# cage-challenge/cage-challenge-4

Hardware: AMD Instinct MI355X
Metric: agent-env steps/sec (5 blue agents x N envs) (higher is better)
Workload: dtype int32

## Files before the change

cage_challenge_4_amd/csrc/cc4_engine.h:

```cpp
#pragma once
#include "cc4_state.h"
#include "cc4_tables.h"

namespace cc4 {

struct Ctx { EnvState* s; EnvCold* c; Rng* r; HostDyn* hd; StepWork* w; unsigned long long* prof = nullptr;
             unsigned long long* aprof = nullptr; EvLog* lg = nullptr; const uint64_t* gpre = nullptr;
             const ExtAct* ext = nullptr; };

#if defined(__HIP_DEVICE_COMPILE__)
#define CC4_TICK(x, i) do { if ((x).prof) { unsigned long long _t = clock64(); (x).prof[(i)] += _t - (x).prof[15]; (x).prof[15] = _t; } } while (0)
#define CC4_TICK0(x) do { if ((x).prof) (x).prof[15] = clock64(); } while (0)
#define CC4_AT0(x) unsigned long long _at = (x).aprof ? clock64() : 0
#define CC4_AT(x, k) do { if ((x).aprof) { unsigned long long _n = clock64(); (x).aprof[(k)] += _n - _at; _at = _n; } } while (0)
#if defined(CC4_FINE)
#define CC4_FT0(x, r) unsigned long long _ft = ((x).aprof && (r) == 0) ? clock64() : 0
#define CC4_FT(x, r, k) do { if ((x).aprof && (r) == 0) { unsigned long long _n = clock64(); (x).aprof[88 + (k)] += _n - _ft; _ft = _n; } } while (0)
#else
#define CC4_FT0(x, r) do { } while (0)
#define CC4_FT(x, r, k) do { } while (0)
#endif
#else
#define CC4_FT0(x, r) do { } while (0)
#define CC4_FT(x, r, k) do { } while (0)
// ... 246 lines not shown
}
CC4_HD void step_red_merge(Ctx x) {
  EnvState* s = x.s;
  uint32_t pr[NRED];
  CC4_UNROLL for (int r = 0; r < NRED; ++r) pr[r] = x.w->pend_r[r];
  CC4_UNROLL for (int r = 0; r < NRED; ++r) {
    if (!pr[r]) continue;
    if (s->npend >= MAX_PEND) set_err(x, E_PEND_OVERFLOW); else s->pend[s->npend++] = pr[r];
    x.w->pend_r[r] = 0;
  }
}
CC4_HD void pend_drop_host(Ctx x, int h) {
  EnvState* s = x.s;
  int n = 0;
  for (int i = 0; i < s->npend; ++i) if ((int)(s->pend[i] >> 16) != h) s->pend[n++] = s->pend[i];
  s->npend = (uint8_t)n;
}
CC4_HD bool subnet_blocked(Ctx x, int src_sub, int other_sub) { return (x.s->blocks[other_sub] >> src_sub) & 1u; }

struct S8 { uint64_t v[8]; uint64_t slots; };
CC4_HD uint64_t rs_word(const EnvState* s, int slot) { uint64_t v; __builtin_memcpy(&v, &s->spool[slot], 8); return v; }
CC4_HD void rs_word_put(EnvState* s, int slot, uint64_t v) { __builtin_memcpy(&s->spool[slot], &v, 8); }
CC4_HD S8 rs_load8(const EnvState* s, const RedAgent& a, int i0) {
  S8 q;
  __builtin_memcpy(&q.slots, &a.sord[i0], 8);
  CC4_UNROLL for (int k = 0; k < 8; ++k) q.v[k] = rs_word(s, (int)((q.slots >> (8 * k)) & 0xFF));
  return q;
}
CC4_HD int s8_slot(const S8& q, int k) { return (int)((q.slots >> (8 * k)) & 0xFF); }
CC4_HD int rsw_id(uint64_t v) { return (int)(v & 0xFFFF); }
CC4_HD int rsw_pid(uint64_t v) { return (int)((v >> 16) & 0xFFFF); }
CC4_HD int rsw_host(uint64_t v) { return (int)((v >> 32) & 0xFF); }
CC4_HD int rsw_flags(uint64_t v) { return (int)((v >> 40) & 0xFF); }
CC4_HD uint64_t rsw_make(int id, int pid, int host, int flags) {
  return (uint64_t)(id & 0xFFFF) | ((uint64_t)(pid & 0xFFFF) << 16) | ((uint64_t)(host & 0xFF) << 32) | ((uint64_t)(flags & 0xFF) << 40);
}
CC4_HD uint64_t rs_at(const EnvState* s, const RedAgent& a, int i) { return rs_word(s, a.sord[i]); }
CC4_HD int rs_find_id(const EnvState* s, const RedAgent& a, int id, int n) {
  for (int i0 = 0; i0 < n; i0 += 8) {
    const S8 q = rs_load8(s, a, i0);
    int hit = -1;
    CC4_UNROLL for (int k = 7; k >= 0; --k) if (i0 + k < n && rsw_id(q.v[k]) == id) hit = i0 + k;
    if (hit >= 0) return hit;
  }
  return -1;
}
CC4_HD int rs_find_id(const EnvState* s, const RedAgent& a, int id) { return rs_find_id(s, a, id, a.h.nsess); }
struct HostSess { int n, first, first_root; };
CC4_HD HostSess rs_on_host(const EnvState* s, const RedAgent& a, int h) {
  HostSess r; r.n = 0; r.first = -1; r.first_root = -1;
  const int n = a.h.nsess;
  for (int i0 = 0; i0 < n; i0 += 8) {
    const S8 q = rs_load8(s, a, i0);
    CC4_UNROLL for (int k = 0; k < 8; ++k)
      if (i0 + k < n && rsw_host(q.v[k]) == h) {
        r.n++;
        if (r.first < 0) r.first = i0 + k;
        if (r.first_root < 0 && (rsw_flags(q.v[k]) & RS_ROOT)) r.first_root = i0 + k;
      }
  }
  return r;
}
CC4_HD int rs_kth_on_host(const EnvState* s, const RedAgent& a, int h, int kth) {
  const int n = a.h.nsess;
  for (int i0 = 0; i0 < n; i0 += 8) {
    const S8 q = rs_load8(s, a, i0);
    int hit = -1;
    CC4_UNROLL for (int k = 0; k < 8; ++k)
      if (hit < 0 && i0 + k < n && rsw_host(q.v[k]) == h) { if (kth == 0) hit = i0 + k; kth--; }
    if (hit >= 0) return hit;
  }
  return -1;
}
CC4_HD int rs_find_host_pid(const EnvState* s, const RedAgent& a, int h, int pid) {
  const int n = a.h.nsess;
  for (int i0 = 0; i0 < n; i0 += 8) {
    const S8 q = rs_load8(s, a, i0);
    int hit = -1;
    CC4_UNROLL for (int k = 7; k >= 0; --k) if (i0 + k < n && rsw_host(q.v[k]) == h && rsw_pid(q.v[k]) == pid) hit = i0 + k;
    if (hit >= 0) return hit;
  }
  return -1;
}
CC4_HD void rs_list_remove(RedAgent& a, int idx) {
  uint64_t w[MAX_RS / 8];
  __builtin_memcpy(w, a.sord, MAX_RS);
  const int wi = idx >> 3, sh = 8 * (idx & 7);
  CC4_UNROLL for (int k = 0; k < MAX_RS / 8; ++k) {
    if (k < wi) continue;
    const uint64_t nxt = k + 1 < MAX_RS / 8 ? w[k + 1] : 0ull;
    uint64_t v = (w[k] >> 8) | (nxt << 56);
    if (k == wi && sh) v = (w[k] & ((1ull << sh) - 1ull)) | (v & ~((1ull << sh) - 1ull));
    w[k] = v;
  }
  __builtin_memcpy(a.sord, w, MAX_RS);
}
CC4_HD int rs_alloc_lowest(Ctx x) {
  for (int w = 0; w < RS_POOL / 32; ++w) {
    const uint32_t fr = ~x.s->spool_used[w];
    if (fr) return w * 32 + ctz32(fr);
  }
  return -1;
}
CC4_HD void rs_reserve(Ctx x) {
  uint32_t used[RS_POOL / 32];
  CC4_UNROLL for (int w = 0; w < RS_POOL / 32; ++w) used[w] = x.s->spool_used[w];
  int ty[NRED];
  CC4_UNROLL for (int r = 0; r < NRED; ++r) ty[r] = x.s->rexec[r].type;
  CC4_UNROLL for (int r = 0; r < NRED; ++r) {
    int slot = 0xFF;
    if (ty[r] == RA_EXPLOIT) {
      CC4_UNROLL for (int w = 0; w < RS_POOL / 32; ++w) {
        const uint32_t fr = ~used[w];
        if (slot == 0xFF && fr) { slot = w * 32 + ctz32(fr); used[w] |= 1u << (slot & 31); }
      }
    }
    x.w->rs_slot[r] = (uint8_t)slot;
  }
}
CC4_HD int rs_add(Ctx x, int r, int host, int pid, int flags, int slot = -1) {
  EnvState* s = x.s;
  RedAgent& a = s->red[r];
  if (slot < 0) slot = rs_alloc_lowest(x);
  if (a.h.nsess >= MAX_RS || slot < 0 || slot >= RS_POOL) { set_err(x, E_RSESS_OVERFLOW); return -1; }
  int id = 0;
  for (int i0 = 0; i0 < a.h.nsess; i0 += 8) {
    const S8 q = rs_load8(s, a, i0);
    CC4_UNROLL for (int k = 0; k < 8; ++k) if (i0 + k < a.h.nsess && rsw_id(q.v[k]) + 1 > id) id = rsw_id(q.v[k]) + 1;
  }
  (void)or_shared(&s->spool_used[slot >> 5], 1u << (slot & 31));
  rs_word_put(s, slot, rsw_make(id, pid, host, flags));
  if (flags & RS_ABSTRACT) {
    uint64_t* row = reinterpret_cast<uint64_t*>(x.c->kports[slot]);
    for (int k = 0; k < (MAXH + 7) / 8; ++k) row[k] = 0;
  }
  a.sord[a.h.nsess++] = (uint8_t)slot;
  a.h.rsc_dirty = 1; a.h.fsm_dirty = 1;
  if (!bit_get(a.live_hosts, host)) { bit_set(a.live_hosts, host); a.h.nlive++; }
  bit_set_shared(s->red_hosts, host);
  return a.h.nsess - 1;
}
CC4_HD void rs_host_left(Ctx x, int r, int gone) {
  RedAgent& a = x.s->red[r];
  bit_clr(a.live_hosts, gone); a.h.nlive--;
  uint32_t lw[NRED];
  CC4_UNROLL for (int q = 0; q < NRED; ++q) lw[q] = x.s->red[q].live_hosts[gone >> 5];
  uint32_t any_other = 0;
  CC4_UNROLL for (int q = 0; q < NRED; ++q) any_other |= lw[q];
  if (!((any_other >> (gone & 31)) & 1u)) bit_clr_shared(x.s->red_hosts, gone);
}
CC4_HD void rs_remove_at(Ctx x, int r, int idx, bool keep_record = false) {
  EnvState* s = x.s;
  RedAgent& a = s->red[r];
  const int slot = a.sord[idx];
  const int gone = rsw_host(rs_word(s, slot));
  if (!keep_record) bit_clr_shared(s->spool_used, slot);
  rs_list_remove(a, idx);
  a.h.nsess--;
  a.h.rsc_dirty = 1; a.h.fsm_dirty = 1;
  if (rs_on_host(s, a, gone).n == 0) rs_host_left(x, r, gone);
}
CC4_HD void rs_remove_on_host(Ctx x, int r, int h) {
  EnvState* s = x.s;
  RedAgent& a = s->red[r];
  const int n = a.h.nsess;
  int out = 0, removed = 0;
// ... 751 lines not shown
    CC4_UNROLL for (int r = 0; r < NRED; ++r) nc += nl[r];
    if (nc == 0) return;
    int c = (int)rng_below(x.r, (uint32_t)nc);
    CC4_UNROLL for (int w = 0; w < 5; ++w) {
      uint32_t m = rh[w];
      if (src >= 0 || !m) continue;
      int inw = 0;
      CC4_UNROLL for (int r = 0; r < NRED; ++r) inw += popc32(lh[r][w]);
      if (c >= inw) { c -= inw; continue; }
      while (m && src < 0) {
        int b = ctz32(m); m &= m - 1;
        CC4_UNROLL for (int r = 0; r < NRED; ++r)
          if (src < 0 && ((lh[r][w] >> b) & 1u)) { if (c-- == 0) src = r; }
      }
    }
  }
  const P8N hd0 = proc_head(x, gh);
  int pid = create_pid(x, gh, hd0);
  if (!add_proc_n(x, gh, hd0.n, pid, K_SESS_RED, 0)) return;
  rs_add(x, src, gh, pid, RS_ABSTRACT);
}
CC4_HD uint64_t green_prepare(Ctx x, int g, int act) {
  EnvState* s = x.s;
  const int gh = s->green_host[g];
  uint64_t w = 0;
  if (act == 1) {
    const HostDyn& d = x.hd[gh];
    uint32_t sv[MAXSV];
    __builtin_memcpy(sv, d.svcs, sizeof(sv));
    const int nsvc = hd_nsvc(d);
    CC4_UNROLL for (int i = 0; i < MAXSV; ++i) if (i < nsvc) w |= (uint64_t)(sv[i] >> 24) << (8 * i);
  } else if (act == 0) {
    uint32_t allowed = green_allowed_mask(s->phase, h_subnet(gh));
    if (x.ext && x.ext[NRED + g].type == XG_ACCESS && x.ext[NRED + g].sid) {
      allowed = (uint32_t)x.ext[NRED + g].sid;
      if (!((allowed >> h_subnet(gh)) & 1u)) allowed = 1u << h_subnet(gh);
    }
    uint64_t ns;
    __builtin_memcpy(&ns, s->n_servers, 8);
    int n = 0;
    CC4_UNROLL for (int sn = 0; sn < NSUB - 1; ++sn) { if ((allowed >> sn) & 1u) n += (int)((ns >> (8 * sn)) & 0xFF); w |= (uint64_t)n << (8 * sn); }
  }
  return w;
}
CC4_HD int green_as_dest(uint64_t pre, int c, int* sn_out) {
  int sn = 0, before = 0;
  CC4_UNROLL for (int k = 0; k < NSUB - 2; ++k) { const int tot = (int)((pre >> (8 * k)) & 0xFF); if (tot <= c) { sn = k + 1; before = tot; } }
  *sn_out = sn;
  return h_make(sn, 11 + (c - before));
}
CC4_HD uint32_t green_lw_active(uint64_t pre) {
  uint32_t act = 0;
  CC4_UNROLL for (int i = 0; i < MAXSV; ++i) if ((pre >> (8 * i)) & SV_ACTIVE) act |= 1u << i;
  return act;
}
CC4_HD bool green_local_work(Ctx x, int gh, uint64_t pre, bool* want_phish, double fp_rate = 0.01, double phish_rate = 0.01) {
  const uint32_t act = green_lw_active(pre);
  if (!act) return false;
  const int c = nth_bit(act, (int)rng_below(x.r, (uint32_t)popc32(act)));
  const uint32_t st = (uint32_t)(pre >> (8 * c)) & 0xFF;
  int rel = (int)(st & 0x7F) * 20;
  if ((int)rng_below(x.r, 100) >= rel) return false;
  if (rng_random_lt(x.r, fp_rate)) { int port = eph_port(x, gh); ev_proc(x, gh, 0); ev_log(x, gh, gh, 1, gh, port, 0xFF, 0, 0); }
  if (rng_random_lt(x.r, phish_rate)) *want_phish = true;
  return true;
}
CC4_HD bool green_access_service(Ctx x, int gh, uint64_t pre, double fp_rate = 0.01) {
  int own = h_subnet(gh);
  const int n = (int)(pre >> 56);
  const int c = (int)rng_below(x.r, (uint32_t)n);
  int sn;
  const int dest = green_as_dest(pre, c, &sn);
  const int dest_port = eph_port(x, dest);
  int ds = sn;
  if (subnet_blocked(x, ds, own) || subnet_blocked(x, own, ds)) { ev_conn(x, dest); ev_log(x, gh, dest, 0, dest, 0, gh, 8800, 0); return false; }
  if (rng_random_lt(x.r, fp_rate)) { ev_conn(x, dest); ev_log(x, gh, dest, 0, gh, 0, dest, dest_port, 0); }
  return true;
}

CC4_HD void red_result(Ctx x, int r, const Act& a, int success) {
  int arg = a.type == RA_DRS ? a.arg : 0;
  obs_first(x, r, success, a.type, a.host, arg);
}
CC4_HD void red_drs(Ctx x, int r, const Act& a) {
  EnvState* s = x.s;
  int sn = a.arg; bool any = false;
  if (rs_find_id(s, s->red[r], a.sid) < 0) { red_result(x, r, a, T_FALSE); return; }
  bool allowed = (red_allowed_mask(r) >> sn) & 1u;
  RedAgent& A = s->red[r];
  const int lo = sn * SLOTS + 1, w0 = lo >> 5, off = lo & 31, w1 = (w0 + 1 < 5) ? w0 + 1 : w0;
  const uint32_t e0 = s->exists[w0], e1 = s->exists[w1], h0 = A.obs_has[1][w0], h1 = A.obs_has[1][w1];
  auto field = [&](uint32_t a0, uint32_t a1) { uint32_t v = a0 >> off; if (off > 16 && w1 != w0) v |= a1 << (32 - off); return v & 0xFFFFu; };
  const uint32_t ex = field(e0, e1);
  any = ex != 0;
  if (allowed && ex) {
    const uint32_t had = field(h0, h1) & ex;
    uint32_t fresh = ex & ~had;
    const uint32_t m0 = ex << off, m1 = (off > 16 && w1 != w0) ? ex >> (32 - off) : 0u;
    A.as_ip[w0] |= m0; A.obs_has[1][w0] = h0 | m0;
    if (m1) { A.as_ip[w1] |= m1; A.obs_has[1][w1] = h1 | m1; }
    A.h.as_subnet |= (uint16_t)(1u << sn);
    int n = A.h.nobs;
    while (fresh) {
      const int b = ctz32(fresh); fresh &= fresh - 1;
      if (n >= MAX_OBS) { set_err(x, E_OBS_OVERFLOW); break; }
      A.obs[n].host = (uint8_t)(lo + b); A.obs[n].flags = (uint8_t)(OE_IFACE | OE_KEY_IP);
      n++;
    }
    A.h.nobs = (uint8_t)n;
    uint32_t again = had;
    while (again) { const int b = ctz32(again); again &= again - 1; obs_put(x, r, true, lo + b, OE_IFACE, true); }
  }
  red_result(x, r, a, any ? T_TRUE : T_UNKNOWN);
}
CC4_HD int port_of_bit(int pb) { return pb == PB_22 ? 22 : (pb == PB_80 ? 80 : (pb == PB_3390 ? 3390 : (pb == PB_25 ? 25 : (pb == PB_1 ? 1 : 443)))); }
CC4_HD void red_scan(Ctx x, int r, const Act& a, double rate) {
  EnvState* s = x.s;
  RedAgent& A = s->red[r];
  int si = rs_find_id(s, A, a.sid);
  if (si < 0) { red_result(x, r, a, T_FALSE); return; }
  const int slot = A.sord[si];
  const uint64_t sw = rs_word(s, slot);
  if (!(rsw_flags(sw) & RS_ABSTRACT)) { red_result(x, r, a, T_FALSE); return; }
  int src = rsw_host(sw), tgt = a.host;
  if (subnet_blocked(x, h_subnet(src), h_subnet(tgt))) { red_result(x, r, a, T_FALSE); return; }
  const bool fixed_le_rate = rng_random_le(x.r, rate);
  int ports = 0;
  const P8N hd0 = proc_head(x, tgt);
  const int np = hd0.n;
  for (int i0 = 0; i0 < np; i0 += 8) {
    P8 q = p8_of(hd0);
    if (i0) q = proc_load8(x, tgt, i0);
    CC4_UNROLL for (int k8 = 0; k8 < 8; ++k8) {
      if (i0 + k8 >= np) continue;
      int k = pw_kind(q.v[k8]);
      int pb = kind_port(k);
      if (!pb) continue;
      ports |= pb;
      if (fixed_le_rate || kind_is_decoy(k)) { ev_conn(x, tgt); int ep = eph_port(x, tgt, (i0 + k8) & 63); ev_log(x, 200 + r, tgt, 0, tgt, port_of_bit(pb), src, ep, 0); }
    }
  }
  if (ports) {
    obs_put(x, r, true, tgt, OE_IFACE, false);
    x.c->kports[slot][tgt] = (uint8_t)(PB_HAS | ports);
  }
  red_result(x, r, a, T_TRUE);
}
CC4_HD int exploit_new_session(Ctx x, int r, int parent_sid, int tgt, const P8N& hd0) {
  (void)parent_sid;
  int pid = create_pid(x, tgt, hd0);
  if (!add_proc_n(x, tgt, hd0.n, pid, K_SHELL, 0)) return -1;
  x.hd[tgt].nsf = (uint8_t)((hd0.nsf & 0x0F) | ((((hd0.nsf >> 4) | HF_CMD) & ~HF_ESC_LAST) << 4));
  return rs_add(x, r, tgt, pid, RS_CHILD, x.w->rs_slot[r]);
}
CC4_HD void red_exploit(Ctx x, int r, const Act& a) {
  EnvState* s = x.s;
  RedAgent& A = s->red[r];
  int si = rs_find_id(s, A, a.sid);
  if (si < 0) { red_result(x, r, a, T_FALSE); return; }
  const int slot = A.sord[si];
  const uint64_t sw = rs_word(s, slot);
  if (!(rsw_flags(sw) & RS_ABSTRACT)) { red_result(x, r, a, T_FALSE); return; }
  int src = rsw_host(sw), tgt = a.host;
  const P8N thd0 = proc_head(x, tgt);
  int known = x.c->kports[slot][tgt];
  if (!(known & PB_HAS)) { red_result(x, r, a, T_FALSE); return; }
  if (subnet_blocked(x, h_subnet(src), h_subnet(tgt))) { red_result(x, r, a, T_FALSE); return; }
  enum { X_HTTPRFI = 0, X_HTTPSRFI = 1, X_SSH = 2, X_SQLI = 3, X_HARAKA = 4 };
  uint32_t opts = 0;
  if (known & PB_80) opts |= 1u << X_HTTPRFI;
  if (known & PB_443) opts |= 1u << X_HTTPSRFI;
  if (known & PB_22) opts |= 1u << X_SSH;
  if ((known & PB_3390) && (known & (PB_80 | PB_443))) opts |= 1u << X_SQLI;
  if (known & PB_25) opts |= 1u << X_HARAKA;
  if (opts == 0) { red_result(x, r, a, T_FALSE); return; }
  int sel = ctz32(opts);
  if (popc32(opts) > 1) {
    int top = (opts >> X_HARAKA) & 1u ? X_HARAKA : ((opts >> X_SQLI) & 1u ? X_SQLI : ((opts >> X_HTTPSRFI) & 1u ? X_HTTPSRFI : X_HTTPRFI));
    opts &= ~(1u << top);
    sel = nth_bit(opts, (int)rng_below(x.r, (uint32_t)popc32(opts)));
    (void)rng_random(x.r);
  }
  const int tnp = thd0.n;
  if (sel == X_SSH) {
    uint8_t* work = reinterpret_cast<uint8_t*>(x.w->scratch + 6 * r);
    int nh = route(src, tgt, work);
    for (int i = 0; i < nh; ++i) if (!rng_random_le(x.r, 0.050000000000000044)) { ev_conn(x, work[12 + i]); ev_log(x, 200 + r, work[12 + i], 0, tgt, 0, src, 22, 0); }
    int vp = -1;
    for (int i0 = 0; i0 < tnp && vp < 0; i0 += 8) {
      P8 q = p8_of(thd0);
      if (i0) q = proc_load8(x, tgt, i0);
      CC4_UNROLL for (int k = 7; k >= 0; --k) if (i0 + k < tnp && pw_kind(q.v[k]) == K_SSHD) vp = i0 + k;
    }
    if (vp < 0) { red_result(x, r, a, T_FALSE); return; }
    obs_put(x, r, true, tgt, OE_IFACE, false);
    const int bf_port = eph_port(x, tgt);
    ev_conn(x, tgt);
    ev_log(x, 200 + r, tgt, 0, tgt, 22, src, bf_port, 0, 10);
    int ni = exploit_new_session(x, r, a.sid, tgt, thd0);
    if (ni < 0) { red_result(x, r, a, T_FALSE); return; }
    const uint64_t nw = rs_at(s, A, ni);
    ev_proc_red(x, r, tgt, rsw_pid(nw));
    ev_log(x, 200 + r, tgt, 1, 0xFF, 0, 0xFF, 0, rsw_pid(nw));
    obs_put(x, r, true, tgt, OE_SESS | OE_IFACE | OE_SYSHN, false);
    obs_put(x, r, true, src, OE_IFACE, false);
    A.h.new_sess_host = (uint8_t)tgt; A.h.new_sess_id = (uint16_t)rsw_id(nw);
    red_result(x, r, a, T_TRUE);
    return;
  }
  int vp = -1, vk = 0;
  {
    const uint32_t want = sel == X_HTTPRFI ? ((1u << K_APACHE) | (1u << K_DEC_APACHE) | (1u << K_DEC_VSFTPD))
                        : sel == X_HTTPSRFI ? (1u << K_DEC_TOMCAT)
                        : sel == X_SQLI ? (1u << K_MYSQL)
                        : ((1u << K_SMTP) | (1u << K_DEC_HARAKA));
    for (int i0 = 0; i0 < tnp && vp < 0; i0 += 8) {
      P8 q = p8_of(thd0);
      if (i0) q = proc_load8(x, tgt, i0);
      CC4_UNROLL for (int k = 7; k >= 0; --k) if (i0 + k < tnp && ((want >> pw_kind(q.v[k])) & 1u)) { vp = i0 + k; vk = pw_kind(q.v[k]); }
    }
  }
  if (vp < 0) { red_result(x, r, a, T_FALSE); return; }
  bool decoy = kind_is_decoy(vk);
  const int xport = sel == X_HTTPRFI ? 80 : (sel == X_HTTPSRFI ? 443 : (sel == X_SQLI ? 3390 : 25));
  if (decoy) { ev_conn(x, tgt); int ep = eph_port(x, tgt, 1); ev_log(x, 200 + r, tgt, 0, tgt, xport, src, ep, 0); }
  obs_put(x, r, true, tgt, OE_IFACE, false);
  bool works = (sel == X_SQLI) || decoy;
  if (!works) { red_result(x, r, a, T_FALSE); return; }
  if (rng_random_le(x.r, 0.0)) { red_result(x, r, a, T_FALSE); return; }
  const int lport = eph_port(x, tgt, 2);
  if (decoy) { ev_conn(x, tgt); int ep = eph_port(x, tgt, 3); ev_log(x, 200 + r, tgt, 0, tgt, lport, src, ep, 0); red_result(x, r, a, T_FALSE); return; }
  int ni = exploit_new_session(x, r, a.sid, tgt, thd0);
  if (ni < 0) { red_result(x, r, a, T_FALSE); return; }
  const uint64_t nw = rs_at(s, A, ni);
  if (!rng_random_le(x.r, 0.050000000000000044)) { ev_proc_red(x, r, tgt, rsw_pid(nw)); ev_log(x, 200 + r, tgt, 1, 0xFF, 0, 0xFF, 0, rsw_pid(nw)); }
  obs_put(x, r, true, tgt, OE_SESS | OE_IFACE | OE_SYSHN, false);
  obs_put(x, r, true, src, OE_IFACE, false);
  A.h.new_sess_host = (uint8_t)tgt; A.h.new_sess_id = (uint16_t)rsw_id(nw);
  red_result(x, r, a, T_TRUE);
}
CC4_HD void red_privesc(Ctx x, int r, const Act& a) {
  EnvState* s = x.s;
  RedAgent& A = s->red[r];
  int h = a.host;
  const HostSess hs = rs_on_host(s, A, h);
  const int n = hs.n;
  int target = hs.first_root;
  if (n == 0) { red_result(x, r, a, T_FALSE); return; }
  if (target < 0) {
    target = rs_kth_on_host(s, A, h, (int)rng_below(x.r, (uint32_t)n));
    { int ss = rs_find_id(s, A, a.sid);
      if (ss < 0 || !(rsw_flags(rs_at(s, A, ss)) & RS_ABSTRACT)) { red_result(x, r, a, T_FALSE); return; } }
    const int tslot = A.sord[target];
    s->spool[tslot].flags |= RS_ROOT;
    hd_touch(x, h);
    hd_set_files(x.hd[h], hd_files(x.hd[h]) | HF_ESC | HF_ESC_LAST);
    int pi = find_proc(x, h, s->spool[tslot].pid);
    if (pi >= 0) proc_put(x, h, pi, proc_get(x, h, pi) | ((uint32_t)PF_ROOT << 24));
  }
  obs_put(x, r, false, h, OE_SESS, false);
  { const uint64_t tw = rs_at(s, A, target); if (rsw_flags(tw) & RS_ABSTRACT) as_know_sid(x, r, rsw_id(tw)); }
  if (rs_find_id(s, A, a.sid) >= 0 && h_slot(h) == 11) {
    uint32_t m = info_links(h_subnet(h));
    for (int sn = 0; sn < NSUB; ++sn) if ((m >> sn) & 1u) obs_put(x, r, false, h_make(sn, 11), OE_IFACE, false);
  }
  red_result(x, r, a, T_TRUE);
}
CC4_HD void red_impact(Ctx x, int r, const Act& a) {
  EnvState* s = x.s;
  RedAgent& A = s->red[r];
  int h = a.host;
  if (rs_on_host(s, A, h).first_root < 0) { red_result(x, r, a, T_FALSE); return; }
  HostDyn& d = x.hd[h];
  const SvTab sv = svc_load(d);
  int si = -1;
  uint32_t sw = 0;
  CC4_UNROLL for (int i = MAXSV - 1; i >= 0; --i) if (i < sv.n && svw_kind(sv.w[i]) == K_OT && (svw_st(sv.w[i]) & SV_ACTIVE)) { si = i; sw = sv.w[i]; }
  if (si < 0) { red_result(x, r, a, T_FALSE); return; }
  if (rs_find_id(s, A, a.sid) < 0) { red_result(x, r, a, T_FALSE); return; }
  hd_touch(x, h);
  d.svcs[si].st = (uint8_t)(svw_st(sw) & ~SV_ACTIVE);
  int pi = find_proc(x, h, (int)(sw & 0xFFFF));
  if (pi >= 0) remove_proc_at(x, h, pi);
  obs_put(x, r, false, h, 0, false);
  red_result(x, r, a, T_TRUE);
}
CC4_HD void red_degrade(Ctx x, int r, const Act& a) {
  EnvState* s = x.s;
  RedAgent& A = s->red[r];
  int h = a.host;
  if (rs_on_host(s, A, h).first_root < 0) { red_result(x, r, a, T_FALSE); return; }
  HostDyn& d = x.hd[h];
  int n = 0;
  hd_touch(x, h);
  const SvTab sv = svc_load(d);
  CC4_UNROLL for (int i = 0; i < MAXSV; ++i) if (i < sv.n && (svw_st(sv.w[i]) & SV_ACTIVE)) {
    n++;
    int rel = svw_st(sv.w[i]) & 0x7F;
    if (rel > 0) rel--;
    d.svcs[i].st = (uint8_t)(SV_ACTIVE | rel);
  }
  if (n == 0) { red_result(x, r, a, T_FALSE); return; }
  obs_put(x, r, false, h, 0, false);
  red_result(x, r, a, T_TRUE);
}
CC4_HD void red_deception(Ctx x, int r, const Act& a) {
  EnvState* s = x.s;
  RedAgent& A = s->red[r];
  if (rs_find_id(s, A, a.sid) < 0) { red_result(x, r, a, T_FALSE); return; }
  int tgt = a.host;
  const double det_rate = (x.ext && (a.busy & AQ_RATE0)) ? x.c->xrate[r][0] : 0.5;
  const double fp_rate = (x.ext && (a.busy & AQ_RATE1)) ? x.c->xrate[r][1] : 0.1;
  const P8N hd0 = proc_head(x, tgt);
  const int np = hd0.n;
  for (int i0 = 0; i0 < np; i0 += 8) {
    P8 q = p8_of(hd0);
    if (i0) q = proc_load8(x, tgt, i0);
    CC4_UNROLL for (int k = 0; k < 8; ++k) {
      if (i0 + k >= np) continue;
      bool decoy = kind_is_decoy(pw_kind(q.v[k]));
      bool rep = false;
      if (rng_random_le(x.r, det_rate) && decoy) rep = true;
      else if (rng_random_le(x.r, fp_rate) && !decoy) rep = true;
      if (rep) obs_put(x, r, false, tgt, OE_IFACE, false);
    }
  }
  red_result(x, r, a, T_TRUE);
}
CC4_HD void red_session_check(Ctx x, int r) {
  EnvState* s = x.s;
  RedAgent& A = s->red[r];
  obs_first(x, r, T_TRUE, RA_NONE, 0, 0);
  if (A.h.nsess == 0) return;
  if (rsw_id(rs_at(s, A, 0)) != 0 && rsw_id(rs_at(s, A, A.h.nsess - 1)) != 0 && rs_find_id(s, A, 0) < 0) {
    int c = (int)rng_below(x.r, (uint32_t)A.h.nsess);
    rs_move_to_end(s, A, c, 0);
    for (int i = 0; i < A.h.nsess; ++i) s->spool[A.sord[i]].flags &= (uint8_t)~RS_CHILD;
  }
  A.h.rsc_listed = 1;
  if (!A.h.rsc_dirty) return;
  const B5 live = b5_load(A.live_hosts);
  { const B5 ip = b5_load(A.as_ip), hn = b5_load(A.as_hn); b5_store(A.as_ip, b5_or(ip, live)); b5_store(A.as_hn, b5_or(hn, live)); }
  {
    uint32_t sub = 0;
    CC4_UNROLL for (int sn = 0; sn < NSUB; ++sn) {
      const int lo = sn * SLOTS, w = lo >> 5, off = lo & 31;
      uint32_t bits = live.w[w] >> off;
      if (off > 32 - SLOTS && w + 1 < 5) bits |= live.w[w + 1] << (32 - off);
      if (bits & ((1u << SLOTS) - 1u)) sub |= 1u << sn;
    }
    A.h.as_subnet |= (uint16_t)sub;
  }
  const int n = A.h.nsess;
  for (int i0 = 0; i0 < n; i0 += 8) {
    const S8 q = rs_load8(s, A, i0);
    uint32_t kw[8];
    CC4_UNROLL for (int k = 0; k < 8; ++k) kw[k] = A.known_bm[(rsw_id(q.v[k]) >> 5) & 7];
    CC4_UNROLL for (int k = 0; k < 8; ++k) {
      if (i0 + k >= n || !(rsw_flags(q.v[k]) & RS_ABSTRACT)) continue;
      const int id = rsw_id(q.v[k]);
      if (id < 256 && ((kw[k] >> (id & 31)) & 1u)) continue;
      as_know_sid(x, r, id);
    }
  }
  A.h.rsc_dirty = 0;
}
CC4_HD void red_withdraw(Ctx x, int r, const Act& a) {
  EnvState* s = x.s;
  RedAgent& A = s->red[r];
  if (rs_find_id(s, A, a.sid) < 0) { red_result(x, r, a, T_FALSE); return; }
  const int h = a.arg;
  uint16_t* ids = reinterpret_cast<uint16_t*>(x.w->scratch + 36);
  int n = 0;
  const int cap = (int)((sizeof(x.w->scratch) - 36 * 4) / 2);
  for (int pass = 0; pass < 2; ++pass)
    for (int i = 0; i < A.h.nsess; ++i) {
      const uint64_t w = rs_at(s, A, i);
      if (rsw_host(w) != h) continue;
      bool child = (rsw_flags(w) & RS_CHILD) != 0;
      if ((pass == 0 && child) || (pass == 1 && !child && rsw_id(w) != 0)) { if (n < cap) ids[n++] = (uint16_t)rsw_id(w); else set_err(x, E_RSESS_OVERFLOW); }
    }
  { int self = rs_find_id(s, A, a.sid); if (rsw_host(rs_at(s, A, self)) == h) { if (n < cap) ids[n++] = (uint16_t)a.sid; else set_err(x, E_RSESS_OVERFLOW); } }
  if (n == 0) { red_result(x, r, a, T_FALSE); return; }
  int ok = T_FALSE;
  for (int k = 0; k < n; ++k) {
    int self = rs_find_id(s, A, a.sid), ti = rs_find_id(s, A, ids[k]);
    if (self < 0 || ti < 0) { ok = T_FALSE; break; }
    int pid = rsw_pid(rs_at(s, A, ti));
    int pi = find_proc(x, h, pid);
    if (pi < 0) { ok = T_FALSE; break; }
    kill_process(x, h, pi, proc_get(x, h, pi));
    ok = T_TRUE;
  }
  red_result(x, r, a, ok);
}
CC4_HD void red_execute(Ctx x, int r, const Act& a) {
  switch (a.type) {
    case RA_DRS: red_drs(x, r, a); break;
    case RA_AGGR: red_scan(x, r, a, (x.ext && (a.busy & AQ_RATE0)) ? x.c->xrate[r][0] : 0.75); break;
    case RA_STEALTH: red_scan(x, r, a, (x.ext && (a.busy & AQ_RATE0)) ? x.c->xrate[r][0] : 0.25); break;
    case RA_DECEPTION: red_deception(x, r, a); break;
    case RA_EXPLOIT: red_exploit(x, r, a); break;
    case RA_PRIVESC: red_privesc(x, r, a); break;
    case RA_IMPACT: red_impact(x, r, a); break;
    case RA_DEGRADE: red_degrade(x, r, a); break;
    case RA_INVALID: obs_first(x, r, T_FALSE, RA_NONE, 0, 0); break;
    case RA_WITHDRAW: red_withdraw(x, r, a); break;
    default: obs_first(x, r, T_UNKNOWN, RA_NONE, 0, 0); break;
  }
}

CC4_HD int fsm_next(int cur, int act, bool success) {
  uint64_t row;
  if (success) switch (cur) {
    case FS_K: row = 0xffffff221ull; break;  case FS_KD: row = 0xffffff331ull; break;
    case FS_S: row = 0xffff42ff3ull; break;  case FS_SD: row = 0xffff53ff3ull; break;
    case FS_U: row = 0x2ff6ffff5ull; break;  case FS_UD: row = 0x3ff7ffff5ull; break;
    case FS_R: row = 0x266fffff7ull; break;  case FS_RD: row = 0x377fffff7ull; break;
    default: row = 0xffffffff8ull; break;
  } else switch (cur) {
    case FS_K: row = 0xffffff000ull; break;  case FS_KD: row = 0xffffff111ull; break;
    case FS_S: row = 0xffff22ff2ull; break;  case FS_SD: row = 0xffff33ff3ull; break;
    case FS_U: row = 0x4ff4ffff4ull; break;  case FS_UD: row = 0x5ff5ffff5ull; break;
    case FS_R: row = 0x666fffff6ull; break;  case FS_RD: row = 0x777fffff7ull; break;
    default: row = 0xffffffff8ull; break;
  }
  int v = (int)((row >> (4 * act)) & 0xF);
  return v == 0xF ? 0xFF : v;
}
CC4_HD int fsm_get(const RedAgent& A, int h) {
  const int v = (A.fsm_st4[h >> 1] >> (4 * (h & 1))) & 0xF;
  return v ? v - 1 : FS_NONE;
}
CC4_HD void fsm_put(RedAgent& A, int h, int st) {
  const int sh = 4 * (h & 1);
  A.fsm_st4[h >> 1] = (uint8_t)((A.fsm_st4[h >> 1] & ~(0xF << sh)) | ((st + 1) << sh));
}
CC4_HD void fsm_set_state(RedAgent& A, int h, int st) {
  if (st >= FS_U && st <= FS_RD) bit_set(A.fsm_ur, h); else bit_clr(A.fsm_ur, h);
  if ((st & 1) || st == FS_F) bit_set(A.fsm_nodrs, h); else bit_clr(A.fsm_nodrs, h);
  fsm_put(A, h, st);
}
CC4_HD void fsm_apply(Ctx x, int r, RedHdr& H, int h, int act, bool success) {
  RedAgent& A = x.s->red[r];
  int cur = fsm_get(A, h);
  if (cur == FS_NONE) return;
  int nx = fsm_next(cur, act, success);
  if (nx == FS_U) nx = ((red_allowed_mask(r) >> h_subnet(h)) & 1u) ? FS_U : FS_F;
  if (nx == 0xFF) nx = cur;
  if (nx != cur) fsm_set_state(A, h, nx);
  if (nx == FS_F && cur != FS_F) {
    int n = 0;
    for (int i = 0; i < H.fsm_n; ++i) if (A.fsm_order[i] != h) A.fsm_order[n++] = A.fsm_order[i];
    H.fsm_n = (uint8_t)n;
  }
}
CC4_HD void fsm_observe(Ctx x, int r, RedHdr& H) {
  RedAgent& A = x.s->red[r];
  CC4_AT0(x);
  if (H.obs_success == T_IN_PROGRESS && H.nobs == 0 && H.rsc_listed && !H.fsm_dirty) return;
  if (H.obs_act_type <= RA_WITHDRAW && H.obs_success != T_IN_PROGRESS && H.obs_success != 0) {
    bool ok = H.obs_success == T_TRUE;
    int t = H.obs_act_type;
    if (t == RA_DRS) {
      const int lo = H.obs_act_arg * SLOTS, hi = lo + SLOTS - 1;
      for (int w = lo >> 5; w <= (hi >> 5) && w < 5; ++w) {
        uint32_t m = A.fsm_known[w];
        if (ok) m &= ~A.fsm_nodrs[w];
        const int l = lo - 32 * w, u = hi - 32 * w;
        if (l > 0) m &= 0xFFFFFFFFu << l;
        if (u < 31) m &= (2u << u) - 1u;
        while (m) { int b = ctz32(m); m &= m - 1; fsm_apply(x, r, H, w * 32 + b, t, ok); }
      }
    } else if (t == RA_PRIVESC || t == RA_IMPACT || t == RA_DEGRADE) {
      int h = H.obs_act_host;
      if (bit_get(A.fsm_known, h) && bit_get(A.fsm_hn, h)) fsm_apply(x, r, H, h, t, ok);
    } else {
      fsm_apply(x, r, H, H.obs_act_host, t, ok);
    }
  }
  CC4_AT(x, 3);
  B5 seen = b5_zero();
  for (int i = 0; i < H.nobs; ++i) {
    int h = A.obs[i].host; int f = A.obs[i].flags;
    if (f & OE_SESS) b5_set(seen, h);
    bool hn = !(f & OE_KEY_IP) || (f & OE_SYSHN);
    bool ip = (f & OE_KEY_IP) || (f & OE_IFACE);
    if (!ip) {
      if (!(bit_get(A.fsm_known, h) && bit_get(A.fsm_hn, h))) { set_err(x, E_UNREACHABLE); }
      continue;
// ... 797 lines not shown
```

cage_challenge_4_amd/csrc/cc4_philox1_body.h:

```cpp
#pragma once
#include "cc4_kernels.h"

#if defined(CC4_EXP_RESET_CALL)
__device__ __attribute__((noinline))
#else
__device__ __forceinline__
#endif
void philox1_autoreset(const StepArgs& a, const int e, const int lane, EnvState* s, HostDyn* const hd, EnvCold* const cold_e, StepWork& work) {
    uint32_t* const ws = a.reset_ws + (size_t)e * RESET_WS_WORDS;
    reset_zero(s, hd, cold_e, lane, WAVE);
    __syncthreads();
    Rng rr; ResetCarry carry; carry.env_key = 0;
    Ctx xm{s, cold_e, &rr, hd, &work};
    if (lane == 0) { rr = s->rng; rr.mode = 1; carry = reset_topology(xm, 0, a.steps, true, a.policy, a.topo, ws, true); }
    __syncthreads();
    Rng rh; rng_fork(&rh, &s->rng, ST_GEN_HOST); rh.mode = 1;
    Ctx xh{s, cold_e, &rh, hd, &work};
    for (int h = lane; h < MAXH; h += WAVE) reset_gen_host(xh, h);
    __syncthreads();
    if (lane == 0) { reset_pid_serial(xm, reset_used_set(s)); reset_agents(xm); }
    __syncthreads();
    reset_used_clear(s, lane, WAVE);
    __syncthreads();
    for (int h = lane; h < MAXH; h += WAVE) reset_host_sessions(xh, h);
// ... 87 lines not shown
      if (is_red) {
        unsigned long long t0 = ap ? clock64() : 0;
        const int dropped = step_red_policy_tick(xr, lane, false, pre_rp);
        if (ap) ap[0] += clock64() - t0;
        if (dropped) atomicSub(&s->n_actions, 1);
      } else if (lane >= 8 && lane < 8 + NBLUE && !(CC4_STOP_ON && a.dbg_stop == 3)) {
        const int b = lane - 8;
        int32_t act = !a.actions ? -1 : a.act_sys ? __hip_atomic_load(a.actions + e * NBLUE + b, __ATOMIC_RELAXED, __HIP_MEMORY_SCOPE_SYSTEM) : a.actions[e * NBLUE + b];
        if (a.rand_out) { act = (int32_t)(((uint64_t)brand * (uint32_t)(b == 4 ? ACT_LONG : ACT_SHORT)) >> 32); a.rand_out[e * NBLUE + b] = act; }
        step_blue_submit(xg, b, act);
        step_tick_blue(xg, b);
        if (!msgs_clean) step_messages(s, a.msgs ? a.msgs + e * NBLUE * MSG_LEN : nullptr, b);
      }
      if (!(CC4_STOP_ON && (a.dbg_stop == 3 || a.dbg_stop == 4))) {
        if (lane < ng) step_green_policy(xg, lane);
        if (lane + WAVE < ng) step_green_policy(xg, lane + WAVE, bank);
      }
      __syncthreads();
      CC4_TICK(x0, 2);
      CC4_STOP(3); CC4_STOP(4); CC4_STOP(5);
      {
        const bool indep = blue_exec_independent(s);
        if (lane == 0) CC4_TICK(x0, 3);
        uint32_t c[4];
        bank_fetch(BK_BEXE, c);
        Ctx xb = xg;
        if (!indep) xb.prof = x0.prof;
        const int rounds = indep ? 1 : 2 * NBLUE;
#pragma nounroll
        for (int i = 0; i < rounds; ++i) {
          int b = lane;
          bool go = lane < NBLUE;
          if (!indep) {
            b = i < NBLUE ? i : i - NBLUE;
            const int ty = s->bexec[b].type;
            go = lane == 0 && ((ty == BA_BLOCK || ty == BA_ALLOW) == (i < NBLUE));
          }
          if (go) {
            rng_set_stream(&rl, ST_BLUE_EXE + (uint32_t)b);
            if (indep) rng_preload(&rl, c);
            blue_execute(xb, b, s->bexec[b]);
          }
        }
        __syncthreads();
        if (lane == 0) CC4_TICK(x0, 5);
      }
      CC4_STOP(6);
      {
        int pen = 0;
        const uint32_t act0 = lane < ng ? work.green_act[lane] : 2u, act1 = lane + WAVE < ng ? work.green_act[lane + WAVE] : 2u;
        const unsigned long long m0 = __ballot(act0 < 2u), m1 = __ballot(act1 < 2u);
        const unsigned long long lt = (1ull << lane) - 1ull;
        const int n0 = __popcll(m0), nact = n0 + __popcll(m1);
        uint8_t* const glist = reinterpret_cast<uint8_t*>(work.scratch);
        static_assert(sizeof(work.scratch) >= MAXG, "the green list fits the scratch words");
        if (act0 < 2u) glist[__popcll(m0 & lt)] = (uint8_t)lane;
        if (act1 < 2u) glist[n0 + __popcll(m1 & lt)] = (uint8_t)(lane + WAVE);
        __syncthreads();
        for (int i = lane; i < nact; i += WAVE) {
          const int g = glist[i];
          uint32_t c[4]; rng_block(&rl, ST_GREEN_EXE + (uint32_t)g, 0, c);
          pen += step_green_exec(xg, g, c);
        }
        if (pen) atomicAdd(&s->brm, pen);
      }
      __syncthreads();
      CC4_TICK(x0, 6);
      CC4_STOP(7);
      if (lane == 0) { step_phishing(x0); CC4_TICK(x0, 1); rs_reserve(x0); conflict_lds = (int)red_conflict_mask(s); if (prof && conflict_lds) prof[4] += 1000000; }
      __syncthreads();
      const uint32_t serial_red = (uint32_t)conflict_lds;
      CC4_STOP(8);
      uint32_t pre_re[4];
      bank_fetch(BK_REXE, pre_re);
      {
        uint32_t todo = serial_red;
        bool side = true;
#pragma nounroll
        for (;;) {
          int r = lane;
          bool go = is_red && !((serial_red >> lane) & 1u);
          Ctx xe = xr;
          if (!side) { r = __ffs((int)todo) - 1; todo &= todo - 1u; go = lane == 0; xe.prof = x0.prof; xe.aprof = nullptr; }
          if (go) {
            unsigned long long t0 = xe.aprof ? clock64() : 0;
            if (s->rexec[r].type != RA_NONE) {
              rng_set_stream(&rl, ST_RED_EXE + (uint32_t)r);
              if (side) rng_preload(&rl, pre_re);
              red_execute(xe, r, s->rexec[r]);
            }
            if (xe.aprof) xe.aprof[1] += clock64() - t0;
          }
          __syncthreads();
          side = false;
          if (!todo) break;
        }
      }
      CC4_STOP(9);
      if (lane == 0) {
        step_red_merge(x0);
        CC4_TICK(x0, 7);
        step_reassign(x0, red_foreign_agents(s));
        CC4_TICK(x0, 8);
      }
      CC4_STOP(10);
      monitor_roll_all(s, lane);
      __syncthreads();
      CC4_TICK(x0, 9);
      CC4_STOP(11);
      if (is_red) { unsigned long long t0 = ap ? clock64() : 0; step_rsc(xr, lane); if (ap) ap[2] += clock64() - t0; }
      if (lane == WAVE - 1) {
        step_monitor_pend(xg);
        step_end(xg, nullptr, false);
        a.reward[e] = s->reward; a.done[e] = s->done;
      }
      CC4_TICK(x0, 10);
    } else if (lane == 0) { a.reward[e] = s->reward; a.done[e] = s->done; }
  }
  __syncthreads();
  CC4_STOP(12);
  unsigned long long t_obs = a.prof ? clock64() : 0;
  {
    int32_t* o = a.obs + (size_t)e * OBS_TOTAL;
    const uint32_t dirty = (do_reset || (a.full_obs && (!PERSIST || item_k == 0))) ? (uint32_t)OD_ALL : (uint32_t)s->obs_dirty;
    encode_obs_fast<WAVE>(s, o, nullptr, false, lane, msgs_clean && !do_reset && dirty != (uint32_t)OD_ALL);
    encode_obs_slow(s, o, dirty, lane);
  }
  __syncthreads();
  CC4_STOP(13);
  if (lane == 0) a.err[e] = s->err;
  unsigned long long t_out = a.prof ? clock64() : 0;
  if (prof && lane == 0) prof[12] += t_out - t_obs;
  if (last) stage_out<HOT_VEC>(reinterpret_cast<uint4*>(a.st + e), lds, lane);
  if (a.obs8) {
    asm volatile("s_waitcnt vmcnt(0)" ::: "memory");
    pack_row_from_obs(a.obs8 + (size_t)e * OBS_PACKED, a.obs + (size_t)e * OBS_TOTAL, lane);
  }
  if (prof && lane == 0) { prof[13] += clock64() - t_out; prof[14] += clock64() - t_begin; }
  if (prof) { __syncthreads(); if (lane < 15) a.prof[PROF_SLOTS * (size_t)e + lane] += prof_lds[lane]; }
}
```

Measured before the change: 1.378 billion.

## Precompute red session lookups cooperatively across the wave before executing red actions

Adds a wave-cooperative query in which groups of 8 lanes scan one red agent's session list in parallel using ballots. From that scan it derives the session index for the action's sid and per-host session counts and first-root positions. The results are passed into each red action handler, replacing that handler's serial per-lane `rs_find_id` and `rs_on_host` scans. This costs an extra wave-wide pass with cross-lane permutes and ballots on the parallel red-execute path, even for agents whose actions never use the lookup.

```diff
diff --git a/cage_challenge_4_amd/csrc/cc4_engine.h b/cage_challenge_4_amd/csrc/cc4_engine.h
--- a/cage_challenge_4_amd/csrc/cc4_engine.h
+++ b/cage_challenge_4_amd/csrc/cc4_engine.h
@@ -352,6 +352,30 @@
   }
   return -1;
 }
+struct RedPre { int si = -1; HostSess hs = {0, -1, -1}; bool ok = false; };
+#if defined(__HIPCC__)
+__device__ __forceinline__ RedPre rs_wave_query(const EnvState* s, int lane, int sid, int host) {
+  const int r = lane >> 3, k = lane & 7, ra = r < NRED ? r : 0;
+  const RedAgent& A = s->red[ra];
+  const int ksid = __builtin_amdgcn_ds_bpermute(ra << 2, sid), khost = __builtin_amdgcn_ds_bpermute(ra << 2, host);
+  const int n = (r < NRED && ksid >= 0) ? (int)A.h.nsess : 0;
+  const int sh = 8 * k;
+  RedPre p; p.ok = true;
+  for (int i0 = 0; __ballot(i0 < n); i0 += 8) {
+    const bool v = i0 + k < n;
+    uint64_t w = 0;
+    if (v) w = rs_word(s, A.sord[i0 + k]);
+    const bool on = v && rsw_host(w) == khost;
+    const uint32_t bid = (uint32_t)(__ballot(v && rsw_id(w) == ksid) >> sh) & 0xFFu;
+    const uint32_t bh = (uint32_t)(__ballot(on) >> sh) & 0xFFu, br = (uint32_t)(__ballot(on && (rsw_flags(w) & RS_ROOT)) >> sh) & 0xFFu;
+    if (p.si < 0 && bid) p.si = i0 + ctz32(bid);
+    p.hs.n += __popc(bh);
+    if (p.hs.first < 0 && bh) p.hs.first = i0 + ctz32(bh);
+    if (p.hs.first_root < 0 && br) p.hs.first_root = i0 + ctz32(br);
+  }
+  return p;
+}
+#endif
 CC4_HD void rs_list_remove(RedAgent& a, int idx) {
   uint64_t w[MAX_RS / 8];
   __builtin_memcpy(w, a.sord, MAX_RS);
@@ -1269,10 +1293,10 @@
   int arg = a.type == RA_DRS ? a.arg : 0;
   obs_first(x, r, success, a.type, a.host, arg);
 }
-CC4_HD void red_drs(Ctx x, int r, const Act& a) {
+CC4_HD void red_drs(Ctx x, int r, const Act& a, RedPre pre = RedPre()) {
   EnvState* s = x.s;
   int sn = a.arg; bool any = false;
-  if (rs_find_id(s, s->red[r], a.sid) < 0) { red_result(x, r, a, T_FALSE); return; }
+  if ((pre.ok ? pre.si : rs_find_id(s, s->red[r], a.sid)) < 0) { red_result(x, r, a, T_FALSE); return; }
   bool allowed = (red_allowed_mask(r) >> sn) & 1u;
   RedAgent& A = s->red[r];
   const int lo = sn * SLOTS + 1, w0 = lo >> 5, off = lo & 31, w1 = (w0 + 1 < 5) ? w0 + 1 : w0;
@@ -1301,10 +1325,10 @@
   red_result(x, r, a, any ? T_TRUE : T_UNKNOWN);
 }
 CC4_HD int port_of_bit(int pb) { return pb == PB_22 ? 22 : (pb == PB_80 ? 80 : (pb == PB_3390 ? 3390 : (pb == PB_25 ? 25 : (pb == PB_1 ? 1 : 443)))); }
-CC4_HD void red_scan(Ctx x, int r, const Act& a, double rate) {
+CC4_HD void red_scan(Ctx x, int r, const Act& a, double rate, RedPre pre = RedPre()) {
   EnvState* s = x.s;
   RedAgent& A = s->red[r];
-  int si = rs_find_id(s, A, a.sid);
+  int si = pre.ok ? pre.si : rs_find_id(s, A, a.sid);
   if (si < 0) { red_result(x, r, a, T_FALSE); return; }
   const int slot = A.sord[si];
   const uint64_t sw = rs_word(s, slot);
@@ -1340,10 +1364,10 @@
   x.hd[tgt].nsf = (uint8_t)((hd0.nsf & 0x0F) | ((((hd0.nsf >> 4) | HF_CMD) & ~HF_ESC_LAST) << 4));
   return rs_add(x, r, tgt, pid, RS_CHILD, x.w->rs_slot[r]);
 }
-CC4_HD void red_exploit(Ctx x, int r, const Act& a) {
+CC4_HD void red_exploit(Ctx x, int r, const Act& a, RedPre pre = RedPre()) {
   EnvState* s = x.s;
   RedAgent& A = s->red[r];
-  int si = rs_find_id(s, A, a.sid);
+  int si = pre.ok ? pre.si : rs_find_id(s, A, a.sid);
   if (si < 0) { red_result(x, r, a, T_FALSE); return; }
   const int slot = A.sord[si];
   const uint64_t sw = rs_word(s, slot);
@@ -1426,17 +1450,17 @@
   A.h.new_sess_host = (uint8_t)tgt; A.h.new_sess_id = (uint16_t)rsw_id(nw);
   red_result(x, r, a, T_TRUE);
 }
-CC4_HD void red_privesc(Ctx x, int r, const Act& a) {
+CC4_HD void red_privesc(Ctx x, int r, const Act& a, RedPre pre = RedPre()) {
   EnvState* s = x.s;
   RedAgent& A = s->red[r];
   int h = a.host;
-  const HostSess hs = rs_on_host(s, A, h);
+  const HostSess hs = pre.ok ? pre.hs : rs_on_host(s, A, h);
   const int n = hs.n;
   int target = hs.first_root;
   if (n == 0) { red_result(x, r, a, T_FALSE); return; }
   if (target < 0) {
     target = rs_kth_on_host(s, A, h, (int)rng_below(x.r, (uint32_t)n));
-    { int ss = rs_find_id(s, A, a.sid);
+    { int ss = pre.ok ? pre.si : rs_find_id(s, A, a.sid);
       if (ss < 0 || !(rsw_flags(rs_at(s, A, ss)) & RS_ABSTRACT)) { red_result(x, r, a, T_FALSE); return; } }
     const int tslot = A.sord[target];
     s->spool[tslot].flags |= RS_ROOT;
@@ -1447,24 +1471,24 @@
   }
   obs_put(x, r, false, h, OE_SESS, false);
   { const uint64_t tw = rs_at(s, A, target); if (rsw_flags(tw) & RS_ABSTRACT) as_know_sid(x, r, rsw_id(tw)); }
-  if (rs_find_id(s, A, a.sid) >= 0 && h_slot(h) == 11) {
+  if ((pre.ok ? pre.si : rs_find_id(s, A, a.sid)) >= 0 && h_slot(h) == 11) {
     uint32_t m = info_links(h_subnet(h));
     for (int sn = 0; sn < NSUB; ++sn) if ((m >> sn) & 1u) obs_put(x, r, false, h_make(sn, 11), OE_IFACE, false);
   }
   red_result(x, r, a, T_TRUE);
 }
-CC4_HD void red_impact(Ctx x, int r, const Act& a) {
+CC4_HD void red_impact(Ctx x, int r, const Act& a, RedPre pre = RedPre()) {
   EnvState* s = x.s;
   RedAgent& A = s->red[r];
   int h = a.host;
-  if (rs_on_host(s, A, h).first_root < 0) { red_result(x, r, a, T_FALSE); return; }
+  if ((pre.ok ? pre.hs : rs_on_host(s, A, h)).first_root < 0) { red_result(x, r, a, T_FALSE); return; }
   HostDyn& d = x.hd[h];
   const SvTab sv = svc_load(d);
   int si = -1;
   uint32_t sw = 0;
   CC4_UNROLL for (int i = MAXSV - 1; i >= 0; --i) if (i < sv.n && svw_kind(sv.w[i]) == K_OT && (svw_st(sv.w[i]) & SV_ACTIVE)) { si = i; sw = sv.w[i]; }
   if (si < 0) { red_result(x, r, a, T_FALSE); return; }
-  if (rs_find_id(s, A, a.sid) < 0) { red_result(x, r, a, T_FALSE); return; }
+  if ((pre.ok ? pre.si : rs_find_id(s, A, a.sid)) < 0) { red_result(x, r, a, T_FALSE); return; }
   hd_touch(x, h);
   d.svcs[si].st = (uint8_t)(svw_st(sw) & ~SV_ACTIVE);
   int pi = find_proc(x, h, (int)(sw & 0xFFFF));
@@ -1472,11 +1496,11 @@
   obs_put(x, r, false, h, 0, false);
   red_result(x, r, a, T_TRUE);
 }
-CC4_HD void red_degrade(Ctx x, int r, const Act& a) {
+CC4_HD void red_degrade(Ctx x, int r, const Act& a, RedPre pre = RedPre()) {
   EnvState* s = x.s;
   RedAgent& A = s->red[r];
   int h = a.host;
-  if (rs_on_host(s, A, h).first_root < 0) { red_result(x, r, a, T_FALSE); return; }
+  if ((pre.ok ? pre.hs : rs_on_host(s, A, h)).first_root < 0) { red_result(x, r, a, T_FALSE); return; }
   HostDyn& d = x.hd[h];
   int n = 0;
   hd_touch(x, h);
@@ -1491,10 +1515,10 @@
   obs_put(x, r, false, h, 0, false);
   red_result(x, r, a, T_TRUE);
 }
-CC4_HD void red_deception(Ctx x, int r, const Act& a) {
+CC4_HD void red_deception(Ctx x, int r, const Act& a, RedPre pre = RedPre()) {
   EnvState* s = x.s;
   RedAgent& A = s->red[r];
-  if (rs_find_id(s, A, a.sid) < 0) { red_result(x, r, a, T_FALSE); return; }
+  if ((pre.ok ? pre.si : rs_find_id(s, A, a.sid)) < 0) { red_result(x, r, a, T_FALSE); return; }
   int tgt = a.host;
   const double det_rate = (x.ext && (a.busy & AQ_RATE0)) ? x.c->xrate[r][0] : 0.5;
   const double fp_rate = (x.ext && (a.busy & AQ_RATE1)) ? x.c->xrate[r][1] : 0.1;
@@ -1552,10 +1576,10 @@
   }
   A.h.rsc_dirty = 0;
 }
-CC4_HD void red_withdraw(Ctx x, int r, const Act& a) {
+CC4_HD void red_withdraw(Ctx x, int r, const Act& a, RedPre pre = RedPre()) {
   EnvState* s = x.s;
   RedAgent& A = s->red[r];
-  if (rs_find_id(s, A, a.sid) < 0) { red_result(x, r, a, T_FALSE); return; }
+  if ((pre.ok ? pre.si : rs_find_id(s, A, a.sid)) < 0) { red_result(x, r, a, T_FALSE); return; }
   const int h = a.arg;
   uint16_t* ids = reinterpret_cast<uint16_t*>(x.w->scratch + 36);
   int n = 0;
@@ -1581,18 +1605,18 @@
   }
   red_result(x, r, a, ok);
 }
-CC4_HD void red_execute(Ctx x, int r, const Act& a) {
+CC4_HD void red_execute(Ctx x, int r, const Act& a, RedPre pre = RedPre()) {
   switch (a.type) {
-    case RA_DRS: red_drs(x, r, a); break;
-    case RA_AGGR: red_scan(x, r, a, (x.ext && (a.busy & AQ_RATE0)) ? x.c->xrate[r][0] : 0.75); break;
-    case RA_STEALTH: red_scan(x, r, a, (x.ext && (a.busy & AQ_RATE0)) ? x.c->xrate[r][0] : 0.25); break;
-    case RA_DECEPTION: red_deception(x, r, a); break;
-    case RA_EXPLOIT: red_exploit(x, r, a); break;
-    case RA_PRIVESC: red_privesc(x, r, a); break;
-    case RA_IMPACT: red_impact(x, r, a); break;
-    case RA_DEGRADE: red_degrade(x, r, a); break;
+    case RA_DRS: red_drs(x, r, a, pre); break;
+    case RA_AGGR: red_scan(x, r, a, (x.ext && (a.busy & AQ_RATE0)) ? x.c->xrate[r][0] : 0.75, pre); break;
+    case RA_STEALTH: red_scan(x, r, a, (x.ext && (a.busy & AQ_RATE0)) ? x.c->xrate[r][0] : 0.25, pre); break;
+    case RA_DECEPTION: red_deception(x, r, a, pre); break;
+    case RA_EXPLOIT: red_exploit(x, r, a, pre); break;
+    case RA_PRIVESC: red_privesc(x, r, a, pre); break;
+    case RA_IMPACT: red_impact(x, r, a, pre); break;
+    case RA_DEGRADE: red_degrade(x, r, a, pre); break;
     case RA_INVALID: obs_first(x, r, T_FALSE, RA_NONE, 0, 0); break;
-    case RA_WITHDRAW: red_withdraw(x, r, a); break;
+    case RA_WITHDRAW: red_withdraw(x, r, a, pre); break;
     default: obs_first(x, r, T_UNKNOWN, RA_NONE, 0, 0); break;
   }
 }
diff --git a/cage_challenge_4_amd/csrc/cc4_philox1_body.h b/cage_challenge_4_amd/csrc/cc4_philox1_body.h
--- a/cage_challenge_4_amd/csrc/cc4_philox1_body.h
+++ b/cage_challenge_4_amd/csrc/cc4_philox1_body.h
@@ -193,12 +193,17 @@
           bool go = is_red && !((serial_red >> lane) & 1u);
           Ctx xe = xr;
           if (!side) { r = __ffs((int)todo) - 1; todo &= todo - 1u; go = lane == 0; xe.prof = x0.prof; xe.aprof = nullptr; }
+          RedPre pe;
+          if (side) {
+            const bool look = go && s->rexec[lane].type < RA_SLEEP;
+            pe = rs_wave_query(s, lane, look ? (int)s->rexec[lane].sid : -1, look ? (int)s->rexec[lane].host : -1);
+          }
           if (go) {
             unsigned long long t0 = xe.aprof ? clock64() : 0;
             if (s->rexec[r].type != RA_NONE) {
               rng_set_stream(&rl, ST_RED_EXE + (uint32_t)r);
               if (side) rng_preload(&rl, pre_re);
-              red_execute(xe, r, s->rexec[r]);
+              red_execute(xe, r, s->rexec[r], pe);
             }
             if (xe.aprof) xe.aprof[1] += clock64() - t0;
           }
```

Result: faster. 1.408 billion, median of 6 (+2.2%).
